# philipturner/metal-flash-attention

Measured on NVIDIA H100. Metric: giga-FMA-instr/sec forward attn N=4096 D=128 bf16, higher is better.
Workload: dtype bf16

## Files before the change

### metal-flash-attention_b200/csrc/kernels/sm90_ptx.cuh

```cuda
#pragma once
#include <cuda_runtime.h>
#include <stdint.h>
#include <stdio.h>

namespace mfa {
namespace ptx {

__device__ __forceinline__ uint32_t smem_u32(const void *p) { return static_cast<uint32_t>(__cvta_generic_to_shared(p)); }

__device__ __forceinline__ uint32_t lane_id() {
  uint32_t r;
  asm volatile("mov.u32 %0, %%laneid;" : "=r"(r));
  return r;
}

__device__ __forceinline__ bool elect_one() {
  uint32_t pred = 0;
  asm volatile(
      "{\n"
      ".reg .pred P;\n"
      "elect.sync _|P, 0xffffffff;\n"
      "selp.u32 %0, 1, 0, P;\n"
      "}\n"
      : "=r"(pred));
  return pred != 0;
}

__device__ __forceinline__ void mbar_init(uint64_t *bar, uint32_t count) {
  asm volatile("mbarrier.init.shared::cta.b64 [%0], %1;" ::"r"(smem_u32(bar)), "r"(count) : "memory");
}
__device__ __forceinline__ void fence_barrier_init() { asm volatile("fence.mbarrier_init.release.cluster;" ::: "memory"); }
__device__ __forceinline__ void fence_proxy_async_smem() { asm volatile("fence.proxy.async.shared::cta;" ::: "memory"); }

__device__ __forceinline__ void mbar_arrive(uint64_t *bar) {
  asm volatile("mbarrier.arrive.shared::cta.b64 _, [%0];" ::"r"(smem_u32(bar)) : "memory");
}
__device__ __forceinline__ void mbar_arrive_expect_tx(uint64_t *bar, uint32_t bytes) {
  asm volatile("mbarrier.arrive.expect_tx.shared::cta.b64 _, [%0], %1;" ::"r"(smem_u32(bar)), "r"(bytes) : "memory");
}
__device__ __forceinline__ bool mbar_try_wait(uint64_t *bar, uint32_t parity) {
  uint32_t ok;
  asm volatile(
      "{\n"
      ".reg .pred P;\n"
      "mbarrier.try_wait.parity.shared::cta.b64 P, [%1], %2;\n"
      "selp.u32 %0, 1, 0, P;\n"
      "}\n"
      : "=r"(ok)
      : "r"(smem_u32(bar)), "r"(parity)
      : "memory");
  return ok != 0;
}

#ifndef MFA_MBAR_TIMEOUT_CYCLES
#define MFA_MBAR_TIMEOUT_CYCLES (8000000000ll)
#endif
__device__ __forceinline__ void mbar_wait(uint64_t *bar, uint32_t parity) {
  if (mbar_try_wait(bar, parity)) return;
  const long long start = clock64();
  uint32_t spins = 0;
  while (!mbar_try_wait(bar, parity)) {
    if ((++spins & 0x3ffu) == 0 && clock64() - start > MFA_MBAR_TIMEOUT_CYCLES) {
      printf("mfa: mbarrier timeout block (%d,%d) thread %d bar@%u parity %u\n", blockIdx.x, blockIdx.y,
             threadIdx.x, smem_u32(bar), parity);
      __trap();
    }
  }
}

__device__ __forceinline__ float4 ldg_stream_f32x4(const float *p) {
  float4 v;
  asm volatile("ld.global.nc.L1::no_allocate.v4.f32 {%0, %1, %2, %3}, [%4];"
               : "=f"(v.x), "=f"(v.y), "=f"(v.z), "=f"(v.w)
               : "l"(p));
  return v;
}
__device__ __forceinline__ uint2 ldg_stream_u32x2(const void *p) {
  uint2 v;
  asm volatile("ld.global.nc.L1::no_allocate.v2.u32 {%0, %1}, [%2];" : "=r"(v.x), "=r"(v.y) : "l"(p));
  return v;
}

__device__ __forceinline__ void prefetch_tensormap(const void *map) {
  asm volatile("prefetch.tensormap [%0];" ::"l"(reinterpret_cast<uint64_t>(map)) : "memory");
}
__device__ __forceinline__ void tma_load_3d(void *smem_dst, const void *map, uint64_t *bar, int32_t c0, int32_t c1,
                                            int32_t c2) {
  asm volatile(
      "cp.async.bulk.tensor.3d.shared::cluster.global.mbarrier::complete_tx::bytes [%0], [%1, {%3, %4, %5}], [%2];"
      ::"r"(smem_u32(smem_dst)), "l"(reinterpret_cast<uint64_t>(map)), "r"(smem_u32(bar)), "r"(c0), "r"(c1), "r"(c2)
      : "memory");
}

__device__ __forceinline__ void tma_store_3d(const void *map, uint32_t smem_src, int32_t c0, int32_t c1, int32_t c2) {
  asm volatile("cp.async.bulk.tensor.3d.global.shared::cta.bulk_group [%0, {%2, %3, %4}], [%1];" ::"l"(
                   reinterpret_cast<uint64_t>(map)),
               "r"(smem_src), "r"(c0), "r"(c1), "r"(c2)
               : "memory");
}
__device__ __forceinline__ void tma_store_commit() { asm volatile("cp.async.bulk.commit_group;" ::: "memory"); }
__device__ __forceinline__ void tma_store_wait_read_all() { asm volatile("cp.async.bulk.wait_group.read 0;" ::: "memory"); }
__device__ __forceinline__ void tma_store_wait_all() { asm volatile("cp.async.bulk.wait_group 0;" ::: "memory"); }

__device__ __forceinline__ void bulk_load_1d(void *smem_dst, const void *gmem_src, uint32_t bytes, uint64_t *bar) {
  asm volatile("cp.async.bulk.shared::cluster.global.mbarrier::complete_tx::bytes [%0], [%1], %2, [%3];" ::"r"(
                   smem_u32(smem_dst)),
               "l"(reinterpret_cast<uint64_t>(gmem_src)), "r"(bytes), "r"(smem_u32(bar))
               : "memory");
}

__device__ __forceinline__ uint64_t make_smem_desc_sw128(uint32_t smem_addr, uint32_t lbo_bytes, uint32_t sbo_bytes) {
  uint64_t desc = 0;
  desc |= static_cast<uint64_t>((smem_addr & 0x3FFFFu) >> 4);
  desc |= static_cast<uint64_t>((lbo_bytes >> 4) & 0x3FFFu) << 16;
  desc |= static_cast<uint64_t>((sbo_bytes >> 4) & 0x3FFFu) << 32;
  desc |= static_cast<uint64_t>(1) << 62;
  return desc;
}

__device__ __forceinline__ void sts_f32x4(uint32_t addr, float4 v) {
  asm volatile("st.shared.v4.f32 [%0], {%1, %2, %3, %4};" ::"r"(addr), "f"(v.x), "f"(v.y), "f"(v.z), "f"(v.w) : "memory");
}
__device__ __forceinline__ float4 lds_f32x4(uint32_t addr) {
  float4 v;
  asm volatile("ld.shared.v4.f32 {%0, %1, %2, %3}, [%4];" : "=f"(v.x), "=f"(v.y), "=f"(v.z), "=f"(v.w) : "r"(addr) : "memory");
  return v;
}

__device__ __forceinline__ float ex2_approx(float x) {
  float y;
  asm("ex2.approx.ftz.f32 %0, %1;" : "=f"(y) : "f"(x));
  return y;
}
__device__ __forceinline__ uint32_t pack_bf16x2(float lo, float hi) {
  uint32_t r;
  asm("cvt.rn.bf16x2.f32 %0, %1, %2;" : "=r"(r) : "f"(hi), "f"(lo));
  return r;
}
__device__ __forceinline__ uint32_t pack_f16x2(float lo, float hi) {
  uint32_t r;
  asm("cvt.rn.f16x2.f32 %0, %1, %2;" : "=r"(r) : "f"(hi), "f"(lo));
  return r;
}

__device__ __forceinline__ float2 unpack_bf16x2(uint32_t w) {
  return make_float2(__uint_as_float(w << 16), __uint_as_float(w & 0xFFFF0000u));
}
__device__ __forceinline__ float2 unpack_f16x2(uint32_t w) {
  float2 r;
  asm("{\n"
      ".reg .b16 lo, hi;\n"
      "mov.b32 {lo, hi}, %2;\n"
      "cvt.f32.f16 %0, lo;\n"
      "cvt.f32.f16 %1, hi;\n"
      "}\n"
      : "=f"(r.x), "=f"(r.y)
      : "r"(w));
  return r;
}

template <uint32_t RegCount>
__device__ __forceinline__ void setmaxnreg_inc() {
  asm volatile("setmaxnreg.inc.sync.aligned.u32 %0;" ::"n"(RegCount));
}
template <uint32_t RegCount>
__device__ __forceinline__ void setmaxnreg_dec() {
  asm volatile("setmaxnreg.dec.sync.aligned.u32 %0;" ::"n"(RegCount));
}

}
}
```

### metal-flash-attention_b200/csrc/kernels/wgmma_attention.cu

```cuda
#include <cuda_fp16.h>
#include <cuda_runtime.h>
#include <math.h>
#include <stdint.h>

#include <type_traits>

#include "attention_params.h"
#include "backward_common.cuh"
#include "device_state.h"
#include "mfa_b200.h"
#include "sm90_ptx.cuh"
#include "tma_host.h"
#include "wgmma.cuh"

namespace mfa {
namespace hop {

using namespace ptx;
using bwd::load_16bit;
using bwd::load_stat;
using bwd::store_stat;

constexpr uint32_t kWG = 128;
constexpr uint32_t kRows = 64;
constexpr uint32_t kBarBytes = 64;

template <uint32_t ROWS>
__device__ __forceinline__ uint64_t desc_kmajor(uint32_t tile, uint32_t row0, uint32_t kk) {
  return make_smem_desc_sw128(tile + (kk >> 2) * ROWS * 128 + row0 * 128 + (kk & 3) * 32, 16, 1024);
}
template <uint32_t ROWS>
__device__ __forceinline__ uint64_t desc_mnmajor(uint32_t tile, uint32_t kk, uint32_t c0) {
  return make_smem_desc_sw128(tile + c0 * ROWS * 128 + kk * 16 * 128, ROWS * 128, 1024);
}

template <bool kBF16>
__device__ __forceinline__ uint32_t pack2(float lo, float hi) {
  return kBF16 ? pack_bf16x2(lo, hi) : pack_f16x2(lo, hi);
}
template <bool kBF16, int NR>
__device__ __forceinline__ void a_frag(const float (&s)[NR], uint32_t kk, uint32_t (&a)[4]) {
  a[0] = pack2<kBF16>(s[8 * kk + 0], s[8 * kk + 1]);
  a[1] = pack2<kBF16>(s[8 * kk + 2], s[8 * kk + 3]);
  a[2] = pack2<kBF16>(s[8 * kk + 4], s[8 * kk + 5]);
  a[3] = pack2<kBF16>(s[8 * kk + 6], s[8 * kk + 7]);
}

__device__ __forceinline__ uint8_t *align1024(uint8_t *p) {
  return reinterpret_cast<uint8_t *>((reinterpret_cast<uintptr_t>(p) + 1023) & ~uintptr_t(1023));
}

template <uint32_t DCH, uint32_t ROWS>
__device__ __forceinline__ void load_tile(uint8_t *dst, const CUtensorMap *map, uint64_t *bar, uint32_t row0,
                                          uint32_t head) {
#pragma unroll
  for (uint32_t c = 0; c < DCH; ++c) tma_load_3d(dst + c * ROWS * 128, map, bar, c * 64, row0, head);
}

template <int N>
__device__ __forceinline__ void zero(float (&d)[N]) {
#pragma unroll
  for (int i = 0; i < N; ++i) d[i] = 0.f;
}

template <int NR>
__device__ __forceinline__ void store_acc(const float (&acc)[NR], float *out, uint32_t row0, uint32_t limit, uint32_t col0,
                                          uint32_t D, float inv0, float inv1) {
  const uint32_t t = threadIdx.x % kWG;
  const uint32_t r = row0 + (t / 32) * 16 + (t % 32) / 4;
#pragma unroll
  for (int i = 0; i < NR / 4; ++i) {
    const uint32_t col = col0 + 8 * i + 2 * (t % 4);
    if (col >= D) continue;
    if (r < limit)
      *reinterpret_cast<float2 *>(out + static_cast<size_t>(r) * D + col) = make_float2(acc[4 * i] * inv0, acc[4 * i + 1] * inv0);
    if (r + 8 < limit)
      *reinterpret_cast<float2 *>(out + static_cast<size_t>(r + 8) * D + col) =
          make_float2(acc[4 * i + 2] * inv1, acc[4 * i + 3] * inv1);
  }
}

struct SplitArgs {
  uint32_t blocks_per_split, splits, batch;
  float *O_part, *L_part;
};

__global__ void __launch_bounds__(128) merge_splits(const SplitArgs sp, float *O, void *L, int l_prec, uint64_t rows_total,
                                                    uint32_t D) {
  const uint64_t idx = static_cast<uint64_t>(blockIdx.x) * blockDim.x + threadIdx.x;
  const uint64_t row = idx / (D / 4);
  if (row >= rows_total) return;
  const uint32_t quad = static_cast<uint32_t>(idx % (D / 4));
  float lmax = -INFINITY;
  for (uint32_t s = 0; s < sp.splits; ++s) lmax = fmaxf(lmax, __ldcg(sp.L_part + s * rows_total + row));
  float denom = 0.f;
  float4 acc = make_float4(0.f, 0.f, 0.f, 0.f);
  for (uint32_t s = 0; s < sp.splits; ++s) {
    const float w = exp2f(__ldcg(sp.L_part + s * rows_total + row) - lmax);
    const float4 v = __ldcg(reinterpret_cast<const float4 *>(sp.O_part + (s * rows_total + row) * D) + quad);
    denom += w;
    acc.x = fmaf(w, v.x, acc.x);
    acc.y = fmaf(w, v.y, acc.y);
    acc.z = fmaf(w, v.z, acc.z);
    acc.w = fmaf(w, v.w, acc.w);
  }
  const float inv = 1.0f / denom;
  *reinterpret_cast<float4 *>(O + row * D + 4 * quad) = make_float4(acc.x * inv, acc.y * inv, acc.z * inv, acc.w * inv);
  if (quad == 0) store_stat(L, row, l_prec, lmax + log2f(denom));
}

template <uint32_t DCH>
struct FwdCfg {
  static constexpr uint32_t kThreads = 2 * kWG, kTileM = 2 * kRows, BN = DCH == 4 ? 64 : 128;
  static constexpr uint32_t kPar = kTileM, kTrav = BN;
  static constexpr uint32_t kQBytes = DCH * kTileM * 128, kKVBytes = DCH * BN * 128;
  static constexpr uint32_t kSmemBytes = 1024 + kQBytes + 2 * 2 * kKVBytes + kBarBytes;
};

template <uint32_t DCH, bool kBF16>
__global__ void __launch_bounds__(2 * kWG, 1)
    attention_forward_wgmma(const __grid_constant__ CUtensorMap mapQ, const __grid_constant__ CUtensorMap mapK,
                            const __grid_constant__ CUtensorMap mapV, float *__restrict__ O, void *__restrict__ L,
                            uint32_t R, uint32_t C, uint32_t D, float scale_log2, int l_prec, const SplitArgs sp) {
  using Cfg = FwdCfg<DCH>;
  constexpr uint32_t NO = DCH * 64, BN = Cfg::BN;
  extern __shared__ uint8_t smem_raw[];
  uint8_t *base = align1024(smem_raw);
  uint8_t *kv = base + Cfg::kQBytes;
  uint64_t *bar = reinterpret_cast<uint64_t *>(kv + 4 * Cfg::kKVBytes);
  const uint32_t tid = threadIdx.x, wg = tid / kWG, t = tid % kWG;
  const uint32_t head = blockIdx.y, row_base = blockIdx.x * Cfg::kTileM;
  const uint32_t kb0 = blockIdx.z * sp.blocks_per_split;
  const uint32_t blocks = min((C + BN - 1) / BN - kb0, sp.blocks_per_split);

  auto load_kv = [&](uint32_t j, uint32_t s) {
    uint8_t *dst = kv + s * 2 * Cfg::kKVBytes;
    mbar_arrive_expect_tx(&bar[1 + s], 2 * Cfg::kKVBytes);
    load_tile<DCH, BN>(dst, &mapK, &bar[1 + s], (kb0 + j) * BN, head);
    load_tile<DCH, BN>(dst + Cfg::kKVBytes, &mapV, &bar[1 + s], (kb0 + j) * BN, head);
  };
  if (tid == 0) {
    prefetch_tensormap(&mapQ);
    prefetch_tensormap(&mapK);
    prefetch_tensormap(&mapV);
    for (int i = 0; i < 3; ++i) mbar_init(&bar[i], 1);
    fence_barrier_init();
  }
  __syncthreads();
  if (tid == 0) {
    mbar_arrive_expect_tx(&bar[0], Cfg::kQBytes);
    load_tile<DCH, Cfg::kTileM>(base, &mapQ, &bar[0], row_base, head);
    for (uint32_t s = 0; s < 2 && s < blocks; ++s) load_kv(s, s);
  }

  const uint32_t sQ = smem_u32(base);
  float o[NO / 2];
  zero(o);
  float m0 = -INFINITY, m1 = -INFINITY, l0 = 0.f, l1 = 0.f;
  mbar_wait(&bar[0], 0);
  for (uint32_t j = 0; j < blocks; ++j) {
    const uint32_t s = j & 1;
    mbar_wait(&bar[1 + s], (j >> 1) & 1);
    const uint32_t sK = smem_u32(kv + s * 2 * Cfg::kKVBytes), sV = sK + Cfg::kKVBytes;
    float sc[BN / 2];
    zero(sc);
    wgmma_fence();
#pragma unroll
    for (uint32_t kk = 0; kk < DCH * 4; ++kk)
      Wgmma<BN, kBF16>::ss(sc, desc_kmajor<Cfg::kTileM>(sQ, wg * kRows, kk), desc_kmajor<BN>(sK, 0, kk), kk > 0);
    wgmma_commit();
    wgmma_wait<0>();
    fence_regs(sc);

    if ((kb0 + j + 1) * BN > C) {
      const uint32_t c0 = (kb0 + j) * BN + 2 * (t % 4);
#pragma unroll
      for (uint32_t i = 0; i < BN / 8; ++i)
#pragma unroll
        for (uint32_t e = 0; e < 2; ++e)
          if (c0 + 8 * i + e >= C) sc[4 * i + e] = sc[4 * i + 2 + e] = -INFINITY;
    }
    float r0 = -INFINITY, r1 = -INFINITY;
#pragma unroll
    for (uint32_t i = 0; i < BN / 8; ++i) {
      r0 = fmaxf(r0, fmaxf(sc[4 * i], sc[4 * i + 1]));
      r1 = fmaxf(r1, fmaxf(sc[4 * i + 2], sc[4 * i + 3]));
    }
    r0 = fmaxf(r0, __shfl_xor_sync(0xffffffffu, r0, 1));
    r0 = fmaxf(r0, __shfl_xor_sync(0xffffffffu, r0, 2));
    r1 = fmaxf(r1, __shfl_xor_sync(0xffffffffu, r1, 1));
    r1 = fmaxf(r1, __shfl_xor_sync(0xffffffffu, r1, 2));
    const float mn0 = fmaxf(m0, r0 * scale_log2), mn1 = fmaxf(m1, r1 * scale_log2);
    const float a0 = ex2_approx(m0 - mn0), a1 = ex2_approx(m1 - mn1);
    m0 = mn0;
    m1 = mn1;
    l0 *= a0;
    l1 *= a1;
#pragma unroll
    for (uint32_t i = 0; i < NO / 8; ++i) {
      o[4 * i] *= a0;
      o[4 * i + 1] *= a0;
      o[4 * i + 2] *= a1;
      o[4 * i + 3] *= a1;
    }
#pragma unroll
    for (uint32_t i = 0; i < BN / 8; ++i) {
      sc[4 * i] = ex2_approx(fmaf(sc[4 * i], scale_log2, -m0));
      sc[4 * i + 1] = ex2_approx(fmaf(sc[4 * i + 1], scale_log2, -m0));
      sc[4 * i + 2] = ex2_approx(fmaf(sc[4 * i + 2], scale_log2, -m1));
      sc[4 * i + 3] = ex2_approx(fmaf(sc[4 * i + 3], scale_log2, -m1));
      l0 += sc[4 * i] + sc[4 * i + 1];
      l1 += sc[4 * i + 2] + sc[4 * i + 3];
    }
    wgmma_fence();
#pragma unroll
    for (uint32_t kk = 0; kk < BN / 16; ++kk) {
      uint32_t a[4];
      a_frag<kBF16>(sc, kk, a);
      Wgmma<NO, kBF16>::rs(o, a, desc_mnmajor<BN>(sV, kk, 0), 1);
    }
    wgmma_commit();
    wgmma_wait<0>();
    fence_regs(o);
    __syncthreads();
    if (tid == 0 && j + 2 < blocks) load_kv(j + 2, s);
  }

  l0 += __shfl_xor_sync(0xffffffffu, l0, 1);
  l0 += __shfl_xor_sync(0xffffffffu, l0, 2);
  l1 += __shfl_xor_sync(0xffffffffu, l1, 1);
  l1 += __shfl_xor_sync(0xffffffffu, l1, 2);
  const uint32_t row0 = row_base + wg * kRows;
  const size_t slice = static_cast<size_t>(blockIdx.z) * sp.batch + head;
  float *Oout = sp.splits == 1 ? O + static_cast<size_t>(head) * R * D : sp.O_part + slice * R * D;
  store_acc(o, Oout, row0, R, 0, D, 1.0f / l0, 1.0f / l1);
  if (t % 4 == 0) {
    const uint32_t r = row0 + (t / 32) * 16 + (t % 32) / 4;
    void *Lout = sp.splits == 1 ? L : sp.L_part;
    const int prec = sp.splits == 1 ? l_prec : FP32;
    const size_t hb = (sp.splits == 1 ? static_cast<size_t>(head) : slice) * R;
    if (r < R) store_stat(Lout, hb + r, prec, m0 + log2f(l0));
    if (r + 8 < R) store_stat(Lout, hb + r + 8, prec, m1 + log2f(l1));
  }
}

template <uint32_t DCH>
struct QCfg {
  static constexpr uint32_t kWarpgroups = DCH == 4 ? 1 : 2;
  static constexpr uint32_t kThreads = kWarpgroups * kWG, kTileM = kWarpgroups * kRows, BN = 64;
  static constexpr uint32_t kPar = kTileM, kTrav = BN;
  static constexpr uint32_t kQBytes = DCH * kTileM * 128, kKVBytes = DCH * BN * 128;
  static constexpr uint32_t kSmemBytes = 1024 + 2 * kQBytes + 2 * 2 * kKVBytes + kBarBytes;
};

struct BwdArgs {
  const float *O;
  const void *dO;
  const void *L;
  void *Dterm;
  float *dQ, *dK, *dV;
  size_t split_stride;
  uint32_t blocks_per_split;
  uint32_t R, C, D;
  float scale, scale_log2;
  int l_prec, d_prec, dO_bf16;
};

template <uint32_t DCH, bool kBF16, bool kConvertDO>
__global__ void __launch_bounds__(QCfg<DCH>::kThreads, 1)
    attention_backward_query_wgmma(const __grid_constant__ CUtensorMap mapQ, const __grid_constant__ CUtensorMap mapdO,
                                   const __grid_constant__ CUtensorMap mapK, const __grid_constant__ CUtensorMap mapV,
                                   const BwdArgs a) {
  using Cfg = QCfg<DCH>;
  constexpr uint32_t NO = DCH * 64, BN = Cfg::BN;
  extern __shared__ uint8_t smem_raw[];
  uint8_t *base = align1024(smem_raw);
  uint8_t *kv = base + 2 * Cfg::kQBytes;
  uint64_t *bar = reinterpret_cast<uint64_t *>(kv + 4 * Cfg::kKVBytes);
  const uint32_t tid = threadIdx.x, wg = tid / kWG, t = tid % kWG;
  const uint32_t head = blockIdx.y, row_base = blockIdx.x * Cfg::kTileM;
  const uint32_t kb0 = blockIdx.z * a.blocks_per_split;
  const uint32_t blocks = min((a.C + BN - 1) / BN - kb0, a.blocks_per_split);

  auto load_kv = [&](uint32_t j, uint32_t s) {
    uint8_t *dst = kv + s * 2 * Cfg::kKVBytes;
    mbar_arrive_expect_tx(&bar[1 + s], 2 * Cfg::kKVBytes);
    load_tile<DCH, BN>(dst, &mapK, &bar[1 + s], (kb0 + j) * BN, head);
    load_tile<DCH, BN>(dst + Cfg::kKVBytes, &mapV, &bar[1 + s], (kb0 + j) * BN, head);
  };
  if (tid == 0) {
    for (int i = 0; i < 3; ++i) mbar_init(&bar[i], 1);
    fence_barrier_init();
  }
  __syncthreads();
  if (tid == 0) {
    mbar_arrive_expect_tx(&bar[0], 2 * Cfg::kQBytes);
    load_tile<DCH, Cfg::kTileM>(base, &mapQ, &bar[0], row_base, head);
    load_tile<DCH, Cfg::kTileM>(base + Cfg::kQBytes, &mapdO, &bar[0], row_base, head);
    for (uint32_t s = 0; s < 2 && s < blocks; ++s) load_kv(s, s);
  }

  const uint32_t row0 = row_base + wg * kRows;
  const uint32_t r = row0 + (t / 32) * 16 + (t % 32) / 4;
  const size_t hb = static_cast<size_t>(head) * a.R;
  float Dr[2], Lr[2];
#pragma unroll
  for (uint32_t h = 0; h < 2; ++h) {
    const uint32_t rc = min(r + 8 * h, a.R - 1);
    const float *Orow = a.O + (hb + rc) * a.D;
    const size_t drow = (hb + rc) * a.D;
    float part = 0.f;
    for (uint32_t d = 2 * (t % 4); d < a.D; d += 8) {
      const float2 ov = *reinterpret_cast<const float2 *>(Orow + d);
      part = fmaf(ov.x, load_16bit(a.dO, drow + d, a.dO_bf16), part);
      part = fmaf(ov.y, load_16bit(a.dO, drow + d + 1, a.dO_bf16), part);
    }
    part += __shfl_xor_sync(0xffffffffu, part, 1);
    part += __shfl_xor_sync(0xffffffffu, part, 2);
    Dr[h] = part * a.scale;
    Lr[h] = load_stat(a.L, hb + rc, a.l_prec);
    if (t % 4 == 0 && r + 8 * h < a.R && blockIdx.z == 0) store_stat(a.Dterm, hb + r + 8 * h, a.d_prec, Dr[h]);
  }

  const uint32_t sQ = smem_u32(base), sdO = sQ + Cfg::kQBytes;
  mbar_wait(&bar[0], 0);
  if constexpr (kConvertDO) {
    uint4 *tile = reinterpret_cast<uint4 *>(base + Cfg::kQBytes);
    for (uint32_t i = tid; i < Cfg::kQBytes / 16; i += Cfg::kThreads) tile[i] = bwd::bf16x8_to_f16x8(tile[i]);
    fence_proxy_async_smem();
    __syncthreads();
  }
  float dq[NO / 2];
  zero(dq);
  for (uint32_t j = 0; j < blocks; ++j) {
    const uint32_t s = j & 1;
    mbar_wait(&bar[1 + s], (j >> 1) & 1);
    const uint32_t sK = smem_u32(kv + s * 2 * Cfg::kKVBytes), sV = sK + Cfg::kKVBytes;
    float sc[BN / 2], dp[BN / 2];
    zero(sc);
    zero(dp);
    wgmma_fence();
#pragma unroll
    for (uint32_t kk = 0; kk < DCH * 4; ++kk)
      Wgmma<BN, kBF16>::ss(sc, desc_kmajor<Cfg::kTileM>(sQ, wg * kRows, kk), desc_kmajor<BN>(sK, 0, kk), kk > 0);
#pragma unroll
    for (uint32_t kk = 0; kk < DCH * 4; ++kk)
      Wgmma<BN, kBF16>::ss(dp, desc_kmajor<Cfg::kTileM>(sdO, wg * kRows, kk), desc_kmajor<BN>(sV, 0, kk), kk > 0);
    wgmma_commit();
    wgmma_wait<0>();
    fence_regs(sc);
    fence_regs(dp);
    const uint32_t c0 = (kb0 + j) * BN + 2 * (t % 4);
#pragma unroll
    for (uint32_t i = 0; i < BN / 8; ++i)
#pragma unroll
      for (uint32_t e = 0; e < 4; ++e) {
        const uint32_t h = e >> 1, k = 4 * i + e;
        const float p = c0 + 8 * i + (e & 1) < a.C ? ex2_approx(fmaf(sc[k], a.scale_log2, -Lr[h])) : 0.f;
        sc[k] = p * fmaf(dp[k], a.scale, -Dr[h]);
      }
    wgmma_fence();
#pragma unroll
    for (uint32_t kk = 0; kk < BN / 16; ++kk) {
      uint32_t f[4];
      a_frag<kBF16>(sc, kk, f);
      Wgmma<NO, kBF16>::rs(dq, f, desc_mnmajor<BN>(sK, kk, 0), 1);
    }
    wgmma_commit();
    wgmma_wait<0>();
    fence_regs(dq);
    __syncthreads();
    if (tid == 0 && j + 2 < blocks) load_kv(j + 2, s);
  }
  store_acc(dq, a.dQ + blockIdx.z * a.split_stride + hb * a.D, row0, a.R, 0, a.D, 1.f, 1.f);
}

template <uint32_t DCH>
struct KVCfg {
  static constexpr bool kSplitD = DCH == 4;
  static constexpr uint32_t kThreads = 2 * kWG, kTileN = kSplitD ? kRows : 2 * kRows, BM = 64;
  static constexpr uint32_t kPar = kTileN, kTrav = BM;
  static constexpr uint32_t kAcc = kSplitD ? 128 : DCH * 64;
  static constexpr uint32_t kKBytes = DCH * kTileN * 128, kQBytes = DCH * BM * 128;
  static constexpr uint32_t kSmemBytes = 1024 + 2 * kKBytes + 2 * 2 * kQBytes + kBarBytes;
};

template <uint32_t DCH, bool kBF16, bool kConvertDO>
__global__ void __launch_bounds__(2 * kWG, 1)
    attention_backward_key_value_wgmma(const __grid_constant__ CUtensorMap mapQ, const __grid_constant__ CUtensorMap mapdO,
                                       const __grid_constant__ CUtensorMap mapK, const __grid_constant__ CUtensorMap mapV,
                                       const BwdArgs a) {
  using Cfg = KVCfg<DCH>;
  constexpr uint32_t BM = Cfg::BM, NA = Cfg::kAcc;
  extern __shared__ uint8_t smem_raw[];
  uint8_t *base = align1024(smem_raw);
  uint8_t *qd = base + 2 * Cfg::kKBytes;
  uint64_t *bar = reinterpret_cast<uint64_t *>(qd + 4 * Cfg::kQBytes);
  const uint32_t tid = threadIdx.x, wg = tid / kWG, t = tid % kWG;
  const uint32_t head = blockIdx.y, key_base = blockIdx.x * Cfg::kTileN;
  const uint32_t qb0 = blockIdx.z * a.blocks_per_split;
  const uint32_t blocks = min((a.R + BM - 1) / BM - qb0, a.blocks_per_split);

  auto load_qd = [&](uint32_t i, uint32_t s) {
    uint8_t *dst = qd + s * 2 * Cfg::kQBytes;
    mbar_arrive_expect_tx(&bar[1 + s], 2 * Cfg::kQBytes);
    load_tile<DCH, BM>(dst, &mapQ, &bar[1 + s], (qb0 + i) * BM, head);
    load_tile<DCH, BM>(dst + Cfg::kQBytes, &mapdO, &bar[1 + s], (qb0 + i) * BM, head);
  };
  if (tid == 0) {
    for (int i = 0; i < 3; ++i) mbar_init(&bar[i], 1);
    fence_barrier_init();
  }
  __syncthreads();
  if (tid == 0) {
    mbar_arrive_expect_tx(&bar[0], 2 * Cfg::kKBytes);
    load_tile<DCH, Cfg::kTileN>(base, &mapK, &bar[0], key_base, head);
    load_tile<DCH, Cfg::kTileN>(base + Cfg::kKBytes, &mapV, &bar[0], key_base, head);
    for (uint32_t s = 0; s < 2 && s < blocks; ++s) load_qd(s, s);
  }
  const uint32_t sK = smem_u32(base), sV = sK + Cfg::kKBytes;
  const uint32_t krow = Cfg::kSplitD ? 0 : wg * kRows;
  const uint32_t nchunk = Cfg::kSplitD ? wg * (NA / 64) : 0;
  const size_t hb = static_cast<size_t>(head) * a.R;
  float dv[NA / 2], dk[NA / 2];
  zero(dv);
  zero(dk);
  mbar_wait(&bar[0], 0);
  for (uint32_t i = 0; i < blocks; ++i) {
    const uint32_t s = i & 1;
    float Lq[BM / 4], Dq[BM / 4];
    const uint32_t q0 = (qb0 + i) * BM + 2 * (t % 4);
#pragma unroll
    for (uint32_t j = 0; j < BM / 8; ++j)
#pragma unroll
      for (uint32_t e = 0; e < 2; ++e) {
        const uint32_t q = min(q0 + 8 * j + e, a.R - 1);
        Lq[2 * j + e] = load_stat(a.L, hb + q, a.l_prec);
        Dq[2 * j + e] = load_stat(a.Dterm, hb + q, a.d_prec);
      }
    mbar_wait(&bar[1 + s], (i >> 1) & 1);
    if constexpr (kConvertDO) {
      uint4 *tile = reinterpret_cast<uint4 *>(qd + s * 2 * Cfg::kQBytes + Cfg::kQBytes);
      for (uint32_t k = tid; k < Cfg::kQBytes / 16; k += Cfg::kThreads) tile[k] = bwd::bf16x8_to_f16x8(tile[k]);
      fence_proxy_async_smem();
      __syncthreads();
    }
    const uint32_t sQ = smem_u32(qd + s * 2 * Cfg::kQBytes), sdO = sQ + Cfg::kQBytes;
    float st[BM / 2], dpt[BM / 2];
    zero(st);
    zero(dpt);
    wgmma_fence();
#pragma unroll
    for (uint32_t kk = 0; kk < DCH * 4; ++kk)
      Wgmma<BM, kBF16>::ss(st, desc_kmajor<Cfg::kTileN>(sK, krow, kk), desc_kmajor<BM>(sQ, 0, kk), kk > 0);
#pragma unroll
    for (uint32_t kk = 0; kk < DCH * 4; ++kk)
      Wgmma<BM, kBF16>::ss(dpt, desc_kmajor<Cfg::kTileN>(sV, krow, kk), desc_kmajor<BM>(sdO, 0, kk), kk > 0);
    wgmma_commit();
    wgmma_wait<0>();
    fence_regs(st);
    fence_regs(dpt);
#pragma unroll
    for (uint32_t j = 0; j < BM / 8; ++j)
#pragma unroll
      for (uint32_t e = 0; e < 4; ++e) {
        const uint32_t k = 4 * j + e, c = 2 * j + (e & 1);
        const float p = q0 + 8 * j + (e & 1) < a.R ? ex2_approx(fmaf(st[k], a.scale_log2, -Lq[c])) : 0.f;
        st[k] = p;
        dpt[k] = p * fmaf(dpt[k], a.scale, -Dq[c]);
      }
    wgmma_fence();
#pragma unroll
    for (uint32_t kk = 0; kk < BM / 16; ++kk) {
      uint32_t f[4];
      a_frag<kBF16>(st, kk, f);
      Wgmma<NA, kBF16>::rs(dv, f, desc_mnmajor<BM>(sdO, kk, nchunk), 1);
      a_frag<kBF16>(dpt, kk, f);
      Wgmma<NA, kBF16>::rs(dk, f, desc_mnmajor<BM>(sQ, kk, nchunk), 1);
    }
    wgmma_commit();
    wgmma_wait<0>();
    fence_regs(dv);
    fence_regs(dk);
    __syncthreads();
    if (tid == 0 && i + 2 < blocks) load_qd(i + 2, s);
  }
  const size_t kb = static_cast<size_t>(head) * a.C * a.D;
  const uint32_t row0 = key_base + krow, col0 = nchunk * 64;
  store_acc(dv, a.dV + blockIdx.z * a.split_stride + kb, row0, a.C, col0, a.D, 1.f, 1.f);
  store_acc(dk, a.dK + blockIdx.z * a.split_stride + kb, row0, a.C, col0, a.D, 1.f, 1.f);
}

static uint32_t chunks(uint32_t D) { return D <= 64 ? 1 : (D <= 128 ? 2 : 4); }

__global__ void __launch_bounds__(256) sum_splits(const float4 *__restrict__ part, float4 *__restrict__ out0,
                                                  float4 *__restrict__ out1, size_t quads, size_t split_stride_quads,
                                                  uint32_t splits) {
  const size_t i = static_cast<size_t>(blockIdx.x) * blockDim.x + threadIdx.x;
  if (i >= quads) return;
  const float4 *src = part + blockIdx.y * quads + i;
  float4 acc = __ldcg(src);
  for (uint32_t s = 1; s < splits; ++s) {
    const float4 v = __ldcg(src + s * split_stride_quads);
    acc.x += v.x;
    acc.y += v.y;
    acc.z += v.z;
    acc.w += v.w;
  }
  (blockIdx.y == 0 ? out0 : out1)[i] = acc;
}

static uint32_t choose_splits(uint32_t items, uint32_t total_blocks, uint32_t sm_count, uint32_t min_blocks,
                              uint32_t max_splits) {
  if (items * 2 > sm_count || min_blocks == 0) return 1;
  if (max_splits > 16) max_splits = 16;
  const uint32_t target = sm_count / items;
  uint32_t best = 1;
  for (uint32_t s = 2; s <= target && s <= max_splits; ++s)
    if (total_blocks % s == 0 && total_blocks / s >= min_blocks) best = s;
  return best;
}

static uint32_t choose_blocks_per_split(uint32_t ctas, uint32_t total_blocks, uint32_t sm_count, uint32_t min_blocks,
                                        uint32_t max_splits) {
  if (ctas * 2 > sm_count || min_blocks == 0 || total_blocks < 2 * min_blocks) return total_blocks;
  if (max_splits > 8) max_splits = 8;
  uint32_t splits = sm_count / ctas;
  if (splits > max_splits) splits = max_splits;
  if (splits < 2) return total_blocks;
  uint32_t per = (total_blocks + splits - 1) / splits;
  if (per < min_blocks) per = min_blocks;
  return per;
}

template <class F>
static auto with_chunks(uint32_t D, F f) {
  switch (chunks(D)) {
    case 1: return f(std::integral_constant<uint32_t, 1>());
    case 2: return f(std::integral_constant<uint32_t, 2>());
    default: return f(std::integral_constant<uint32_t, 4>());
  }
}

template <typename Kernel>
static cudaError_t prepare(Kernel kernel, uint32_t smem) {
  return ensure_max_dynamic_smem(reinterpret_cast<const void *>(kernel), smem, current_device());
}

template <uint32_t DCH, bool kBF16>
cudaError_t launch_forward(const AttentionParams &p, const WgmmaPlan &plan, cudaStream_t stream) {
  using Cfg = FwdCfg<DCH>;
  auto kernel = attention_forward_wgmma<DCH, kBF16>;
  cudaError_t e;
  if ((e = prepare(kernel, Cfg::kSmemBytes)) != cudaSuccess) return e;
  CUtensorMap mapQ, mapK, mapV;
  if ((e = make_tensor_map_16bit(&mapQ, p.buf[sQ], p.R, p.D, p.batch, Cfg::kTileM)) != cudaSuccess) return e;
  if ((e = make_tensor_map_16bit(&mapK, p.buf[sK], p.C, p.D, p.batch, Cfg::BN)) != cudaSuccess) return e;
  if ((e = make_tensor_map_16bit(&mapV, p.buf[sV], p.C, p.D, p.batch, Cfg::BN)) != cudaSuccess) return e;
  SplitArgs sp{plan.blocks_per_split, plan.splits, p.batch, nullptr, nullptr};
  const uint64_t rows_total = static_cast<uint64_t>(p.batch) * p.R;
  if (plan.splits > 1) {
    void *ws = nullptr;
    const size_t o_elems = plan.splits * rows_total * p.D;
    if ((e = workspace_for(current_device(), stream, (o_elems + plan.splits * rows_total) * sizeof(float), &ws)) !=
        cudaSuccess)
      return e;
    sp.O_part = static_cast<float *>(ws);
    sp.L_part = sp.O_part + o_elems;
  }
  kernel<<<plan.grid, Cfg::kThreads, Cfg::kSmemBytes, stream>>>(mapQ, mapK, mapV, static_cast<float *>(p.buf[sO]),
                                                                p.buf[sL], p.R, p.C, p.D, p.scale_log2, p.prec[sL], sp);
  if ((e = cudaGetLastError()) != cudaSuccess || plan.splits == 1) return e;
  const uint64_t threads = rows_total * (p.D / 4);
  merge_splits<<<static_cast<uint32_t>((threads + 127) / 128), 128, 0, stream>>>(sp, static_cast<float *>(p.buf[sO]),
                                                                                 p.buf[sL], p.prec[sL], rows_total, p.D);
  return cudaGetLastError();
}

static cudaError_t split_scratch(BwdArgs &a, uint32_t splits, uint32_t tensors, size_t tensor_elems, cudaStream_t stream,
                                 float **scratch) {
  void *ws = nullptr;
  cudaError_t e = workspace_for(current_device(), stream, splits * tensors * tensor_elems * sizeof(float), &ws);
  if (e != cudaSuccess) return e;
  *scratch = static_cast<float *>(ws);
  a.split_stride = tensors * tensor_elems;
  return cudaSuccess;
}

static cudaError_t launch_sum(const float *scratch, float *out0, float *out1, size_t tensor_elems, uint32_t tensors,
                              size_t split_stride, uint32_t splits, cudaStream_t stream) {
  const size_t quads = tensor_elems / 4;
  sum_splits<<<dim3(static_cast<uint32_t>((quads + 255) / 256), tensors), 256, 0, stream>>>(
      reinterpret_cast<const float4 *>(scratch), reinterpret_cast<float4 *>(out0), reinterpret_cast<float4 *>(out1), quads,
      split_stride / 4, splits);
  return cudaGetLastError();
}

static BwdArgs backward_args(const AttentionParams &p, const WgmmaPlan &plan) {
  BwdArgs a;
  a.O = static_cast<const float *>(p.buf[sO]);
  a.dO = p.buf[sdO];
  a.L = p.buf[sL];
  a.Dterm = p.buf[sD];
  a.dQ = static_cast<float *>(p.buf[sdQ]);
  a.dK = static_cast<float *>(p.buf[sdK]);
  a.dV = static_cast<float *>(p.buf[sdV]);
  a.blocks_per_split = plan.blocks_per_split;
  a.R = p.R;
  a.C = p.C;
  a.D = p.D;
  a.scale = p.scale;
  a.scale_log2 = p.scale_log2;
  a.l_prec = p.prec[sL];
  a.d_prec = p.prec[sD];
  a.dO_bf16 = p.prec[sdO] == BF16;
  return a;
}

template <uint32_t DCH, bool kBF16, bool kConvertDO>
cudaError_t launch_query(const AttentionParams &p, const WgmmaPlan &plan, cudaStream_t stream) {
  using Cfg = QCfg<DCH>;
  auto kernel = attention_backward_query_wgmma<DCH, kBF16, kConvertDO>;
  cudaError_t e;
  if ((e = prepare(kernel, Cfg::kSmemBytes)) != cudaSuccess) return e;
  CUtensorMap mapQ, mapdO, mapK, mapV;
  if ((e = make_tensor_map_16bit(&mapQ, p.buf[sQ], p.R, p.D, p.batch, Cfg::kTileM)) != cudaSuccess) return e;
  if ((e = make_tensor_map_16bit(&mapdO, p.buf[sdO], p.R, p.D, p.batch, Cfg::kTileM)) != cudaSuccess) return e;
  if ((e = make_tensor_map_16bit(&mapK, p.buf[sK], p.C, p.D, p.batch, Cfg::BN)) != cudaSuccess) return e;
  if ((e = make_tensor_map_16bit(&mapV, p.buf[sV], p.C, p.D, p.batch, Cfg::BN)) != cudaSuccess) return e;
  BwdArgs a = backward_args(p, plan);
  const size_t tensor_elems = static_cast<size_t>(p.batch) * p.R * p.D;
  float *scratch = nullptr;
  if (plan.splits > 1) {
    if ((e = split_scratch(a, plan.splits, 1, tensor_elems, stream, &scratch)) != cudaSuccess) return e;
    a.dQ = scratch;
  }
  kernel<<<plan.grid, Cfg::kThreads, Cfg::kSmemBytes, stream>>>(mapQ, mapdO, mapK, mapV, a);
  if ((e = cudaGetLastError()) != cudaSuccess || plan.splits == 1) return e;
  return launch_sum(scratch, static_cast<float *>(p.buf[sdQ]), nullptr, tensor_elems, 1, a.split_stride, plan.splits,
                    stream);
}

template <uint32_t DCH, bool kBF16, bool kConvertDO>
cudaError_t launch_key_value(const AttentionParams &p, const WgmmaPlan &plan, cudaStream_t stream) {
  using Cfg = KVCfg<DCH>;
  auto kernel = attention_backward_key_value_wgmma<DCH, kBF16, kConvertDO>;
  cudaError_t e;
  if ((e = prepare(kernel, Cfg::kSmemBytes)) != cudaSuccess) return e;
  CUtensorMap mapQ, mapdO, mapK, mapV;
  if ((e = make_tensor_map_16bit(&mapQ, p.buf[sQ], p.R, p.D, p.batch, Cfg::BM)) != cudaSuccess) return e;
  if ((e = make_tensor_map_16bit(&mapdO, p.buf[sdO], p.R, p.D, p.batch, Cfg::BM)) != cudaSuccess) return e;
  if ((e = make_tensor_map_16bit(&mapK, p.buf[sK], p.C, p.D, p.batch, Cfg::kTileN)) != cudaSuccess) return e;
  if ((e = make_tensor_map_16bit(&mapV, p.buf[sV], p.C, p.D, p.batch, Cfg::kTileN)) != cudaSuccess) return e;
  BwdArgs a = backward_args(p, plan);
  const size_t tensor_elems = static_cast<size_t>(p.batch) * p.C * p.D;
  float *scratch = nullptr;
  if (plan.splits > 1) {
    if ((e = split_scratch(a, plan.splits, 2, tensor_elems, stream, &scratch)) != cudaSuccess) return e;
    a.dV = scratch;
    a.dK = scratch + tensor_elems;
  }
  kernel<<<plan.grid, Cfg::kThreads, Cfg::kSmemBytes, stream>>>(mapQ, mapdO, mapK, mapV, a);
  if ((e = cudaGetLastError()) != cudaSuccess || plan.splits == 1) return e;
  return launch_sum(scratch, static_cast<float *>(p.buf[sdV]), static_cast<float *>(p.buf[sdK]), tensor_elems, 2,
                    a.split_stride, plan.splits, stream);
}

template <class F>
static cudaError_t dispatch(const AttentionParams &p, bool convert_dO, F f) {
  return with_chunks(p.D, [&](auto dch) {
    if (convert_dO) return f(dch, std::false_type(), std::true_type());
    if (p.prec[sQ] == BF16) return f(dch, std::true_type(), std::false_type());
    return f(dch, std::false_type(), std::false_type());
  });
}

}

WgmmaPlan wgmma_plan(int type, uint32_t D, uint32_t R, uint32_t C, uint32_t batch, uint32_t min_blocks,
                     uint32_t max_splits, bool convert_dO, uint32_t sm_count) {
  WgmmaPlan p{};
  auto geometry = [&](auto cfg) {
    using Cfg = decltype(cfg);
    p.threads = Cfg::kThreads;
    p.smem_bytes = Cfg::kSmemBytes;
    p.par = Cfg::kPar;
    p.trav = Cfg::kTrav;
  };
  hop::with_chunks(D, [&](auto dch) {
    constexpr uint32_t DCH = decltype(dch)::value;
    if (type == MFA_FORWARD)
      geometry(hop::FwdCfg<DCH>());
    else if (type == MFA_BACKWARD_QUERY)
      geometry(hop::QCfg<DCH>());
    else
      geometry(hop::KVCfg<DCH>());
  });
  const uint32_t padded = (D + 7) / 8 * 8, columns = hop::chunks(D) * 64;
  p.head = columns < padded ? columns : padded;

  const bool key_value = type == MFA_BACKWARD_KEY_VALUE;
  const uint32_t tiles = ((key_value ? C : R) + p.par - 1) / p.par, total = ((key_value ? R : C) + p.trav - 1) / p.trav;
  if (type == MFA_FORWARD) {
    p.splits = hop::choose_splits(tiles * batch, total, sm_count, min_blocks, max_splits);
    p.blocks_per_split = total / p.splits;
  } else {
    p.blocks_per_split = hop::choose_blocks_per_split(tiles * batch, total, sm_count, min_blocks, max_splits);
    p.splits = (total + p.blocks_per_split - 1) / p.blocks_per_split;
  }
  p.grid = dim3(tiles, batch, p.splits);
  p.convert_dO_first = key_value && convert_dO && static_cast<uint64_t>(tiles) * batch > sm_count;
  p.launches = 1 + (p.splits > 1 ? 1 : 0) + (p.convert_dO_first ? 1 : 0);
  return p;
}

static bool row_major_16bit(const AttentionParams &p) {
  for (int s = 0; s < kSlots; ++s)
    if (p.transposed[s]) return false;
  return (p.prec[sQ] == FP16 || p.prec[sQ] == BF16) && p.prec[sK] == p.prec[sQ] && p.prec[sV] == p.prec[sQ] &&
         p.D % 8 == 0 && p.D <= kWgmmaMaxHead;
}

static WgmmaPlan plan_for(int type, const AttentionParams &p, bool convert_dO) {
  return wgmma_plan(type, p.D, p.R, p.C, p.batch, p.split_min_blocks, p.split_max, convert_dO,
                    device_sm_count(current_device()));
}

cudaError_t launch_wgmma_forward(const AttentionParams &p, cudaStream_t stream) {
  if (!row_major_16bit(p) || p.prec[sO] != FP32) {
    set_launch_detail("descriptor is outside the wgmma forward kernel's domain");
    return cudaErrorInvalidValue;
  }
  const WgmmaPlan plan = plan_for(MFA_FORWARD, p, false);
  return hop::dispatch(p, false, [&](auto dch, auto bf16, auto) {
    return hop::launch_forward<decltype(dch)::value, decltype(bf16)::value>(p, plan, stream);
  });
}

static bool backward_ok(const AttentionParams &p) {
  const bool dO_ok = p.prec[sdO] == p.prec[sQ] || (p.prec[sQ] == FP16 && p.prec[sdO] == BF16);
  return row_major_16bit(p) && dO_ok && p.prec[sO] == FP32 && p.prec[sdQ] == FP32 && p.prec[sdK] == FP32 &&
         p.prec[sdV] == FP32;
}

cudaError_t launch_wgmma_backward_query(const AttentionParams &p, cudaStream_t stream) {
  if (!backward_ok(p)) {
    set_launch_detail("descriptor is outside the wgmma backward kernels' domain");
    return cudaErrorInvalidValue;
  }
  const bool convert = p.prec[sdO] != p.prec[sQ];
  const WgmmaPlan plan = plan_for(MFA_BACKWARD_QUERY, p, convert);
  return hop::dispatch(p, convert, [&](auto dch, auto bf16, auto cvt) {
    return hop::launch_query<decltype(dch)::value, decltype(bf16)::value, decltype(cvt)::value>(p, plan, stream);
  });
}

cudaError_t launch_wgmma_backward_key_value(const AttentionParams &p, cudaStream_t stream) {
  if (!backward_ok(p)) {
    set_launch_detail("descriptor is outside the wgmma backward kernels' domain");
    return cudaErrorInvalidValue;
  }
  const bool convert = p.prec[sdO] != p.prec[sQ];
  const WgmmaPlan plan = plan_for(MFA_BACKWARD_KEY_VALUE, p, convert);
  AttentionParams q = p;
  if (plan.convert_dO_first) {
    const uint64_t elements = static_cast<uint64_t>(p.batch) * p.R * p.D;
    void *converted = nullptr;
    cudaError_t e = workspace_for(current_device(), stream, elements * 2, &converted, 2);
    if (e != cudaSuccess) return e;
    if ((e = launch_bf16_to_f16(p.buf[sdO], converted, elements, stream)) != cudaSuccess) return e;
    q.buf[sdO] = converted;
    q.prec[sdO] = q.prec[sQ];
  }
  return hop::dispatch(q, convert && !plan.convert_dO_first, [&](auto dch, auto bf16, auto cvt) {
    return hop::launch_key_value<decltype(dch)::value, decltype(bf16)::value, decltype(cvt)::value>(q, plan, stream);
  });
}

}
```

Before: 223,100.

## Add ping-pong warpgroup scheduling with split K/V barriers and deeper pipeline

Measured after the change: 228,100, median of 6. 1.02x the previous value.

```diff
diff --git a/metal-flash-attention_b200/csrc/kernels/sm90_ptx.cuh b/metal-flash-attention_b200/csrc/kernels/sm90_ptx.cuh
--- a/metal-flash-attention_b200/csrc/kernels/sm90_ptx.cuh
+++ b/metal-flash-attention_b200/csrc/kernels/sm90_ptx.cuh
@@ -55,17 +55,28 @@
 #ifndef MFA_MBAR_TIMEOUT_CYCLES
 #define MFA_MBAR_TIMEOUT_CYCLES (8000000000ll)
 #endif
+template <bool kReport = true>
 __device__ __forceinline__ void mbar_wait(uint64_t *bar, uint32_t parity) {
   if (mbar_try_wait(bar, parity)) return;
   const long long start = clock64();
   uint32_t spins = 0;
   while (!mbar_try_wait(bar, parity)) {
     if ((++spins & 0x3ffu) == 0 && clock64() - start > MFA_MBAR_TIMEOUT_CYCLES) {
-      printf("mfa: mbarrier timeout block (%d,%d) thread %d bar@%u parity %u\n", blockIdx.x, blockIdx.y,
-             threadIdx.x, smem_u32(bar), parity);
+      if (kReport)
+        printf("mfa: mbarrier timeout block (%d,%d) thread %d bar@%u parity %u\n", blockIdx.x, blockIdx.y,
+               threadIdx.x, smem_u32(bar), parity);
       __trap();
     }
   }
+}
+
+template <uint32_t kId, uint32_t kCount>
+__device__ __forceinline__ void named_bar_sync() {
+  asm volatile("bar.sync %0, %1;" ::"n"(kId), "n"(kCount) : "memory");
+}
+template <uint32_t kId, uint32_t kCount>
+__device__ __forceinline__ void named_bar_arrive() {
+  asm volatile("bar.arrive %0, %1;" ::"n"(kId), "n"(kCount) : "memory");
 }
 
 __device__ __forceinline__ float4 ldg_stream_f32x4(const float *p) {
diff --git a/metal-flash-attention_b200/csrc/kernels/wgmma_attention.cu b/metal-flash-attention_b200/csrc/kernels/wgmma_attention.cu
--- a/metal-flash-attention_b200/csrc/kernels/wgmma_attention.cu
+++ b/metal-flash-attention_b200/csrc/kernels/wgmma_attention.cu
@@ -113,9 +113,52 @@
 struct FwdCfg {
   static constexpr uint32_t kThreads = 2 * kWG, kTileM = 2 * kRows, BN = DCH == 4 ? 64 : 128;
   static constexpr uint32_t kPar = kTileM, kTrav = BN;
+  static constexpr uint32_t kStages = DCH == 4 ? 2 : 3;
+  static constexpr bool kPingPong = DCH != 4;
   static constexpr uint32_t kQBytes = DCH * kTileM * 128, kKVBytes = DCH * BN * 128;
-  static constexpr uint32_t kSmemBytes = 1024 + kQBytes + 2 * 2 * kKVBytes + kBarBytes;
+  static constexpr uint32_t kBarBytes = 128;
+  static constexpr uint32_t kSmemBytes = 1024 + kQBytes + kStages * 2 * kKVBytes + kBarBytes;
+  static_assert((1 + 4 * kStages) * 8 <= kBarBytes, "mbarriers do not fit");
 };
+
+template <uint32_t BN>
+__device__ __forceinline__ void online_softmax(float (&sc)[BN / 2], uint32_t key0, uint32_t C, float scale_log2,
+                                               float &m0, float &m1, float &l0, float &l1, float &a0, float &a1) {
+  if (key0 + BN > C) {
+    const uint32_t c0 = key0 + 2 * (threadIdx.x % 4);
+#pragma unroll
+    for (uint32_t i = 0; i < BN / 8; ++i)
+#pragma unroll
+      for (uint32_t e = 0; e < 2; ++e)
+        if (c0 + 8 * i + e >= C) sc[4 * i + e] = sc[4 * i + 2 + e] = -INFINITY;
+  }
+  float r0 = -INFINITY, r1 = -INFINITY;
+#pragma unroll
+  for (uint32_t i = 0; i < BN / 8; ++i) {
+    r0 = fmaxf(r0, fmaxf(sc[4 * i], sc[4 * i + 1]));
+    r1 = fmaxf(r1, fmaxf(sc[4 * i + 2], sc[4 * i + 3]));
+  }
+  r0 = fmaxf(r0, __shfl_xor_sync(0xffffffffu, r0, 1));
+  r0 = fmaxf(r0, __shfl_xor_sync(0xffffffffu, r0, 2));
+  r1 = fmaxf(r1, __shfl_xor_sync(0xffffffffu, r1, 1));
+  r1 = fmaxf(r1, __shfl_xor_sync(0xffffffffu, r1, 2));
+  const float mn0 = fmaxf(m0, r0 * scale_log2), mn1 = fmaxf(m1, r1 * scale_log2);
+  a0 = ex2_approx(m0 - mn0);
+  a1 = ex2_approx(m1 - mn1);
+  m0 = mn0;
+  m1 = mn1;
+  l0 *= a0;
+  l1 *= a1;
+#pragma unroll
+  for (uint32_t i = 0; i < BN / 8; ++i) {
+    sc[4 * i] = ex2_approx(fmaf(sc[4 * i], scale_log2, -m0));
+    sc[4 * i + 1] = ex2_approx(fmaf(sc[4 * i + 1], scale_log2, -m0));
+    sc[4 * i + 2] = ex2_approx(fmaf(sc[4 * i + 2], scale_log2, -m1));
+    sc[4 * i + 3] = ex2_approx(fmaf(sc[4 * i + 3], scale_log2, -m1));
+    l0 += sc[4 * i] + sc[4 * i + 1];
+    l1 += sc[4 * i + 2] + sc[4 * i + 3];
+  }
+}
 
 template <uint32_t DCH, bool kBF16>
 __global__ void __launch_bounds__(2 * kWG, 1)
@@ -123,107 +166,169 @@
                             const __grid_constant__ CUtensorMap mapV, float *__restrict__ O, void *__restrict__ L,
                             uint32_t R, uint32_t C, uint32_t D, float scale_log2, int l_prec, const SplitArgs sp) {
   using Cfg = FwdCfg<DCH>;
-  constexpr uint32_t NO = DCH * 64, BN = Cfg::BN;
+  constexpr uint32_t NO = DCH * 64, BN = Cfg::BN, S = Cfg::kStages;
   extern __shared__ uint8_t smem_raw[];
   uint8_t *base = align1024(smem_raw);
   uint8_t *kv = base + Cfg::kQBytes;
-  uint64_t *bar = reinterpret_cast<uint64_t *>(kv + 4 * Cfg::kKVBytes);
+  uint64_t *bar = reinterpret_cast<uint64_t *>(kv + S * 2 * Cfg::kKVBytes);
+  uint64_t *k_full = bar + 1, *v_full = bar + 1 + S;
+  uint64_t *k_free = bar + 1 + 2 * S, *v_free = bar + 1 + 3 * S;
   const uint32_t tid = threadIdx.x, wg = tid / kWG, t = tid % kWG;
   const uint32_t head = blockIdx.y, row_base = blockIdx.x * Cfg::kTileM;
   const uint32_t kb0 = blockIdx.z * sp.blocks_per_split;
   const uint32_t blocks = min((C + BN - 1) / BN - kb0, sp.blocks_per_split);
 
-  auto load_kv = [&](uint32_t j, uint32_t s) {
-    uint8_t *dst = kv + s * 2 * Cfg::kKVBytes;
-    mbar_arrive_expect_tx(&bar[1 + s], 2 * Cfg::kKVBytes);
-    load_tile<DCH, BN>(dst, &mapK, &bar[1 + s], (kb0 + j) * BN, head);
-    load_tile<DCH, BN>(dst + Cfg::kKVBytes, &mapV, &bar[1 + s], (kb0 + j) * BN, head);
+  auto load = [&](uint32_t v, uint32_t j) {
+    const uint32_t s = j % S;
+    uint64_t *full = v ? &v_full[s] : &k_full[s];
+    mbar_arrive_expect_tx(full, Cfg::kKVBytes);
+    load_tile<DCH, BN>(kv + (2 * s + v) * Cfg::kKVBytes, v ? &mapV : &mapK, full, (kb0 + j) * BN, head);
   };
   if (tid == 0) {
     prefetch_tensormap(&mapQ);
     prefetch_tensormap(&mapK);
     prefetch_tensormap(&mapV);
-    for (int i = 0; i < 3; ++i) mbar_init(&bar[i], 1);
+    mbar_init(&bar[0], 1);
+    for (uint32_t s = 0; s < S; ++s) {
+      mbar_init(&k_full[s], 1);
+      mbar_init(&v_full[s], 1);
+      mbar_init(&k_free[s], 2);
+      mbar_init(&v_free[s], 2);
+    }
     fence_barrier_init();
   }
   __syncthreads();
   if (tid == 0) {
     mbar_arrive_expect_tx(&bar[0], Cfg::kQBytes);
     load_tile<DCH, Cfg::kTileM>(base, &mapQ, &bar[0], row_base, head);
-    for (uint32_t s = 0; s < 2 && s < blocks; ++s) load_kv(s, s);
+    for (uint32_t j = 0; j < S && j < blocks; ++j) {
+      load(0, j);
+      load(1, j);
+    }
   }
 
   const uint32_t sQ = smem_u32(base);
-  float o[NO / 2];
+  auto stage_k = [&](uint32_t s) { return smem_u32(kv + s * 2 * Cfg::kKVBytes); };
+  float o[NO / 2], sc[BN / 2];
+  uint32_t p[BN / 16][4];
   zero(o);
-  float m0 = -INFINITY, m1 = -INFINITY, l0 = 0.f, l1 = 0.f;
-  mbar_wait(&bar[0], 0);
-  for (uint32_t j = 0; j < blocks; ++j) {
-    const uint32_t s = j & 1;
-    mbar_wait(&bar[1 + s], (j >> 1) & 1);
-    const uint32_t sK = smem_u32(kv + s * 2 * Cfg::kKVBytes), sV = sK + Cfg::kKVBytes;
-    float sc[BN / 2];
-    zero(sc);
+  zero(sc);
+  float m0 = -INFINITY, m1 = -INFINITY, l0 = 0.f, l1 = 0.f, a0, a1;
+  auto issue_s = [&](uint32_t s) {
+#pragma unroll
+    for (uint32_t kk = 0; kk < DCH * 4; ++kk)
+      Wgmma<BN, kBF16>::ss(sc, desc_kmajor<Cfg::kTileM>(sQ, wg * kRows, kk), desc_kmajor<BN>(stage_k(s), 0, kk), kk > 0);
+    wgmma_commit();
+  };
+  auto issue_pv = [&](uint32_t s) {
+#pragma unroll
+    for (uint32_t kk = 0; kk < BN / 16; ++kk)
+      Wgmma<NO, kBF16>::rs(o, p[kk], desc_mnmajor<BN>(stage_k(s) + Cfg::kKVBytes, kk, 0), 1);
+    wgmma_commit();
+  };
+  auto pack_p = [&] {
+#pragma unroll
+    for (uint32_t kk = 0; kk < BN / 16; ++kk) a_frag<kBF16>(sc, kk, p[kk]);
+  };
+  auto release = [&](uint32_t v, uint32_t j) {
+    if (t != 0) return;
+    uint64_t *free = v ? &v_free[j % S] : &k_free[j % S];
+    mbar_arrive(free);
+    if (wg == 1 && j + S < blocks) {
+      mbar_wait<false>(free, (j / S) & 1);
+      load(v, j + S);
+    }
+  };
+  auto turn_begin = [&] {
+    if (wg == 0)
+      named_bar_sync<1, 2 * kWG>();
+    else
+      named_bar_sync<2, 2 * kWG>();
+  };
+  auto turn_end = [&] {
+    if (wg == 0)
+      named_bar_arrive<2, 2 * kWG>();
+    else
+      named_bar_arrive<1, 2 * kWG>();
+  };
+  mbar_wait<false>(&bar[0], 0);
+  if constexpr (!Cfg::kPingPong) {
+    for (uint32_t j = 0; j < blocks; ++j) {
+      const uint32_t s = j % S;
+      mbar_wait<false>(&k_full[s], (j / S) & 1);
+      wgmma_fence();
+      issue_s(s);
+      wgmma_wait<0>();
+      fence_regs(sc);
+      online_softmax<BN>(sc, (kb0 + j) * BN, C, scale_log2, m0, m1, l0, l1, a0, a1);
+#pragma unroll
+      for (uint32_t i = 0; i < NO / 8; ++i) {
+        o[4 * i] *= a0;
+        o[4 * i + 1] *= a0;
+        o[4 * i + 2] *= a1;
+        o[4 * i + 3] *= a1;
+      }
+      pack_p();
+      mbar_wait<false>(&v_full[s], (j / S) & 1);
+      wgmma_fence();
+      issue_pv(s);
+      wgmma_wait<0>();
+      fence_regs(o);
+      __syncthreads();
+      if (tid == 0 && j + S < blocks) {
+        load(0, j + S);
+        load(1, j + S);
+      }
+    }
+  } else {
+    if (wg == 1) turn_end();
+
+    mbar_wait<false>(&k_full[0], 0);
+    turn_begin();
     wgmma_fence();
-#pragma unroll
-    for (uint32_t kk = 0; kk < DCH * 4; ++kk)
-      Wgmma<BN, kBF16>::ss(sc, desc_kmajor<Cfg::kTileM>(sQ, wg * kRows, kk), desc_kmajor<BN>(sK, 0, kk), kk > 0);
-    wgmma_commit();
+    issue_s(0);
+    turn_end();
     wgmma_wait<0>();
     fence_regs(sc);
-
-    if ((kb0 + j + 1) * BN > C) {
-      const uint32_t c0 = (kb0 + j) * BN + 2 * (t % 4);
-#pragma unroll
-      for (uint32_t i = 0; i < BN / 8; ++i)
-#pragma unroll
-        for (uint32_t e = 0; e < 2; ++e)
-          if (c0 + 8 * i + e >= C) sc[4 * i + e] = sc[4 * i + 2 + e] = -INFINITY;
-    }
-    float r0 = -INFINITY, r1 = -INFINITY;
-#pragma unroll
-    for (uint32_t i = 0; i < BN / 8; ++i) {
-      r0 = fmaxf(r0, fmaxf(sc[4 * i], sc[4 * i + 1]));
-      r1 = fmaxf(r1, fmaxf(sc[4 * i + 2], sc[4 * i + 3]));
-    }
-    r0 = fmaxf(r0, __shfl_xor_sync(0xffffffffu, r0, 1));
-    r0 = fmaxf(r0, __shfl_xor_sync(0xffffffffu, r0, 2));
-    r1 = fmaxf(r1, __shfl_xor_sync(0xffffffffu, r1, 1));
-    r1 = fmaxf(r1, __shfl_xor_sync(0xffffffffu, r1, 2));
-    const float mn0 = fmaxf(m0, r0 * scale_log2), mn1 = fmaxf(m1, r1 * scale_log2);
-    const float a0 = ex2_approx(m0 - mn0), a1 = ex2_approx(m1 - mn1);
-    m0 = mn0;
-    m1 = mn1;
-    l0 *= a0;
-    l1 *= a1;
-#pragma unroll
-    for (uint32_t i = 0; i < NO / 8; ++i) {
-      o[4 * i] *= a0;
-      o[4 * i + 1] *= a0;
-      o[4 * i + 2] *= a1;
-      o[4 * i + 3] *= a1;
-    }
-#pragma unroll
-    for (uint32_t i = 0; i < BN / 8; ++i) {
-      sc[4 * i] = ex2_approx(fmaf(sc[4 * i], scale_log2, -m0));
-      sc[4 * i + 1] = ex2_approx(fmaf(sc[4 * i + 1], scale_log2, -m0));
-      sc[4 * i + 2] = ex2_approx(fmaf(sc[4 * i + 2], scale_log2, -m1));
-      sc[4 * i + 3] = ex2_approx(fmaf(sc[4 * i + 3], scale_log2, -m1));
-      l0 += sc[4 * i] + sc[4 * i + 1];
-      l1 += sc[4 * i + 2] + sc[4 * i + 3];
-    }
-    wgmma_fence();
-#pragma unroll
-    for (uint32_t kk = 0; kk < BN / 16; ++kk) {
-      uint32_t a[4];
-      a_frag<kBF16>(sc, kk, a);
-      Wgmma<NO, kBF16>::rs(o, a, desc_mnmajor<BN>(sV, kk, 0), 1);
-    }
-    wgmma_commit();
-    wgmma_wait<0>();
-    fence_regs(o);
-    __syncthreads();
-    if (tid == 0 && j + 2 < blocks) load_kv(j + 2, s);
+    release(0, 0);
+    online_softmax<BN>(sc, kb0 * BN, C, scale_log2, m0, m1, l0, l1, a0, a1);
+    pack_p();
+    for (uint32_t j = 0; j + 1 < blocks; ++j) {
+      const uint32_t s = j % S, sn = (j + 1) % S;
+      mbar_wait<false>(&k_full[sn], ((j + 1) / S) & 1);
+      mbar_wait<false>(&v_full[s], (j / S) & 1);
+      turn_begin();
+      wgmma_fence();
+      issue_s(sn);
+      issue_pv(s);
+      turn_end();
+      wgmma_wait<1>();
+      fence_regs(sc);
+      online_softmax<BN>(sc, (kb0 + j + 1) * BN, C, scale_log2, m0, m1, l0, l1, a0, a1);
+      wgmma_wait<0>();
+      fence_regs(o);
+      release(0, j + 1);
+      release(1, j);
+#pragma unroll
+      for (uint32_t i = 0; i < NO / 8; ++i) {
+        o[4 * i] *= a0;
+        o[4 * i + 1] *= a0;
+        o[4 * i + 2] *= a1;
+        o[4 * i + 3] *= a1;
+      }
+      pack_p();
+    }
+    {
+      const uint32_t s = (blocks - 1) % S;
+      mbar_wait<false>(&v_full[s], ((blocks - 1) / S) & 1);
+      turn_begin();
+      wgmma_fence();
+      issue_pv(s);
+      turn_end();
+      if (wg == 0) named_bar_sync<1, 2 * kWG>();
+      wgmma_wait<0>();
+      fence_regs(o);
+    }
   }
 
   l0 += __shfl_xor_sync(0xffffffffu, l0, 1);
```
